# eragonruan/text-detection-ctpn

Hardware: AMD Instinct MI355X
Metric: images/sec at 600x900 (VGG16-CTPN inference) (higher is better)
Workload: dtype bf16

## Files before the change

text-detection-ctpn_amd/csrc/conv3x3_impl.h:

```cpp
#pragma once
#include <cstdlib>
#include <mutex>
#include <type_traits>
#include <utility>

#include "common.h"

namespace ctpn {

constexpr int C3_MAX_DEV = CTPN_MAX_DEV;
static inline int c3_device(int& dev) { return current_device(dev); }
static inline int c3_cu_count(int dev, int& ncu) { return device_cu_count(dev, ncu); }
static inline int c3_raise_lds(const void* kern, bool (&done)[C3_MAX_DEV], int dev) { return raise_dynamic_lds(kern, 160 * 1024, done, dev); }

typedef ctpn_f32x16 c3_f32x16;
typedef __attribute__((ext_vector_type(4))) float c3_f32x4;
typedef uint32_t c3_u32x4 __attribute__((ext_vector_type(4)));

template <typename T>
__device__ __forceinline__ void c3_mfma(c3_f32x16& acc, const uint4& w, const uint4& x) {
  if constexpr (std::is_same<T, float>::value) {
    acc = __builtin_amdgcn_mfma_f32_32x32x2f32(__builtin_bit_cast(float, w.x), __builtin_bit_cast(float, x.x), acc, 0, 0, 0);
    acc = __builtin_amdgcn_mfma_f32_32x32x2f32(__builtin_bit_cast(float, w.y), __builtin_bit_cast(float, x.y), acc, 0, 0, 0);
    acc = __builtin_amdgcn_mfma_f32_32x32x2f32(__builtin_bit_cast(float, w.z), __builtin_bit_cast(float, x.z), acc, 0, 0, 0);
// ... 865 lines not shown
          const uint32_t offA = (uint32_t)((wm * (Wo + 2) + xa) * opitch) * 2u;
          store_pair(pb + (size_t)offA, rok && (cur.x0 >> 1) + xa < Wo, pb + (size_t)offA + (size_t)(8 * opitch) * 2u, rok && (cur.x0 >> 1) + xb < Wo, true, mine);
        } else {
          const int Xl = lq >> 1;
          const uint32_t loff = (uint32_t)((wm * (Wo + 2) + Xl) * opitch) * (uint32_t)sizeof(OutT);
          store_tile(pb + (size_t)loff, !odd && (cur.y0 >> 1) + wm < Ho && (cur.x0 >> 1) + Xl < Wo && ch0 < g.Co, mine);
        }
      } else if constexpr (TW == 32) {
        c3_f32x16 v0, v1;
#pragma unroll
        for (int r = 0; r < 16; ++r) { v0[r] = __builtin_fmaxf(acc[0][0][r], acc[0][1][r]); v1[r] = __builtin_fmaxf(acc[NTL - 1][0][r], acc[NTL - 1][1][r]); }
        hpool(v0, v1, wm, lq >> 1, true);
      } else {
        const int vpart = ((lane & 32) | ((lq & 16) ? ((lq - 2) & 15) : 16 + ((lq + 2) & 15))) << 2;
#pragma unroll
        for (int j = 0; j < MT; ++j) {
          c3_f32x16 v0, v1;
#pragma unroll
          for (int r = 0; r < 16; ++r) {
            const float a0 = acc[0][j][r], a1 = acc[NTL - 1][j][r];
            float b0 = __builtin_bit_cast(float, __builtin_amdgcn_ds_bpermute(vpart, __builtin_bit_cast(int, a0)));
            float b1 = __builtin_bit_cast(float, __builtin_amdgcn_ds_bpermute(vpart, __builtin_bit_cast(int, a1)));
            asm volatile("" : "+v"(b0), "+v"(b1));
            v0[r] = __builtin_fmaxf(a0, b0); v1[r] = __builtin_fmaxf(a1, b1);
          }
          hpool(v0, v1, wm * MT + j, (lq & 15) >> 1, (lq & 16) == 0);
        }
      }
    }
    if (!has_next) break;
    lid = nlid;
    cur = nxt;
    cur_tile = nxt_tile; cur_half = nxt_half;
    if constexpr (HT) active = cur_half < 0 || wm < 2;
  }
  c3_wait_vm<0>();
}

struct Conv3WR {
  const void* in; const void* wt; const float* bias; void* out; void* pool_out;
  int N, H, W, Co;
  int tiles_x, tiles_y, tiles_n;
  unsigned ptiles;
  unsigned groups, per_group;
  unsigned magic_img, magic_row;
  char* dump;
  unsigned* claim;
  const void* q; const void* wfq;
  int Hq, Wq;
};

constexpr int WR_PITCH = 144, WR_PW = 34, WR_ROWS = 10 * WR_PW, WR_PIECES = 48, WR_WIN = WR_PIECES * 1024, WR_NBUF = 3, WR_PD = 8;
static_assert(WR_ROWS * WR_PITCH <= WR_WIN, "window must fit its pieces");

template <int... I, typename F>
__device__ __forceinline__ void c3_static_for_impl(std::integer_sequence<int, I...>, F&& f) { (f(std::integral_constant<int, I>{}), ...); }
template <int N, typename F>
__device__ __forceinline__ void c3_static_for(F&& f) { c3_static_for_impl(std::make_integer_sequence<int, N>{}, f); }

template <int OFF, bool XA = false>
__device__ __forceinline__ void c3_ds_read_b128_off(c3_u32x4& dst, uint32_t lds_addr) {
  if constexpr (XA) asm volatile("ds_read_b128 %0, %1 offset:%2" : "+a"(dst) : "v"(lds_addr), "n"(OFF));
  else asm volatile("ds_read_b128 %0, %1 offset:%2" : "+v"(dst) : "v"(lds_addr), "n"(OFF));
}
#define C3_DEFINE_SLOTS(SFX, MN, XC) \
template <int OFF, int WAIT, int INIT> \
__device__ __forceinline__ void c3_slot1##SFX(c3_f32x16& a0, const c3_u32x4& w0, c3_u32x4& x, uint32_t xaddr, const c3_f32x16& bias) { \
  if constexpr (INIT == 0) \
    asm volatile("s_waitcnt lgkmcnt(%6)\n\t" MN "%0, %2, %1, %3\n\tds_read_b128 %1, %4 offset:%5" \
                 : "+v"(a0), XC(x) : "a"(w0), "v"(bias), "v"(xaddr), "n"(OFF), "n"(WAIT)); \
  else \
    asm volatile("s_waitcnt lgkmcnt(%5)\n\t" MN "%0, %2, %1, %0\n\tds_read_b128 %1, %3 offset:%4" \
                 : "+v"(a0), XC(x) : "a"(w0), "v"(xaddr), "n"(OFF), "n"(WAIT)); \
} \
template <int OFF, int WAIT, int INIT> \
__device__ __forceinline__ void c3_slot2##SFX(c3_f32x16& a0, c3_f32x16& a1, const c3_u32x4& w0, const c3_u32x4& w1, c3_u32x4& x, uint32_t xaddr, \
                                         const c3_f32x16& bias) { \
  if constexpr (INIT == 0) \
    asm volatile("s_waitcnt lgkmcnt(%8)\n\t" MN "%0, %3, %2, %5\n\t" MN "%1, %4, %2, %1\n\tds_read_b128 %2, %6 offset:%7" \
                 : "+v"(a0), "+v"(a1), XC(x) : "a"(w0), "a"(w1), "v"(bias), "v"(xaddr), "n"(OFF), "n"(WAIT)); \
  else if constexpr (INIT == 1) \
    asm volatile("s_waitcnt lgkmcnt(%8)\n\t" MN "%0, %3, %2, %0\n\t" MN "%1, %4, %2, %5\n\tds_read_b128 %2, %6 offset:%7" \
                 : "+v"(a0), "+v"(a1), XC(x) : "a"(w0), "a"(w1), "v"(bias), "v"(xaddr), "n"(OFF), "n"(WAIT)); \
  else \
    asm volatile("s_waitcnt lgkmcnt(%7)\n\t" MN "%0, %3, %2, %0\n\t" MN "%1, %4, %2, %1\n\tds_read_b128 %2, %5 offset:%6" \
                 : "+v"(a0), "+v"(a1), XC(x) : "a"(w0), "a"(w1), "v"(xaddr), "n"(OFF), "n"(WAIT)); \
} \
template <int OFF, int WAIT> \
__device__ __forceinline__ void c3_slot3##SFX(c3_f32x16& a0, c3_f32x16& a1, c3_f32x16& a2, const c3_u32x4& w0, const c3_u32x4& w1, const c3_u32x4& w2, \
                                         c3_u32x4& x, uint32_t xaddr) { \
  asm volatile("s_waitcnt lgkmcnt(%9)\n\t" MN "%0, %4, %3, %0\n\t" MN "%1, %5, %3, %1\n\t" MN "%2, %6, %3, %2\n\tds_read_b128 %3, %7 offset:%8" \
               : "+v"(a0), "+v"(a1), "+v"(a2), XC(x) : "a"(w0), "a"(w1), "a"(w2), "v"(xaddr), "n"(OFF), "n"(WAIT)); \
}
C3_DEFINE_SLOTS(_bf16, "v_mfma_f32_32x32x16_bf16 ", "+v")
C3_DEFINE_SLOTS(_f16, "v_mfma_f32_32x32x16_f16 ", "+v")
C3_DEFINE_SLOTS(_bf16a, "v_mfma_f32_32x32x16_bf16 ", "+a")
C3_DEFINE_SLOTS(_f16a, "v_mfma_f32_32x32x16_f16 ", "+a")
#undef C3_DEFINE_SLOTS
template <bool F16, bool XA, int OFF, int WAIT, int INIT>
__device__ __forceinline__ void c3_slot1(c3_f32x16& a0, const c3_u32x4& w0, c3_u32x4& x, uint32_t xaddr, const c3_f32x16& bias) {
  if constexpr (F16 && XA) c3_slot1_f16a<OFF, WAIT, INIT>(a0, w0, x, xaddr, bias);
  else if constexpr (F16) c3_slot1_f16<OFF, WAIT, INIT>(a0, w0, x, xaddr, bias);
  else if constexpr (XA) c3_slot1_bf16a<OFF, WAIT, INIT>(a0, w0, x, xaddr, bias);
  else c3_slot1_bf16<OFF, WAIT, INIT>(a0, w0, x, xaddr, bias);
}
template <bool F16, bool XA, int OFF, int WAIT, int INIT>
// ... 44 lines not shown
  return w > 15 ? 15 : w;
}

__host__ __device__ constexpr int fq_slot_of(int kind, int id) {
  for (int n = 0; n < 72; ++n)
    if ((kind == 0 ? fq_setup(n) : kind == 1 ? fq_read(n) : kind == 2 ? fq_mma(n) : fq_epi(n)) == id) return n;
  return -1;
}
__host__ __device__ constexpr bool fq_schedule_ok() {
  for (int n = 0; n < 72; ++n) {
    if (fq_lds_ops(n) > 1) return false;
    if ((fq_setup(n) >= 0 || fq_lds_ops(n) || fq_mma(n) >= 0) && (n <= WR_PD || n > 69)) return false;
  }
  if (!(FQ_INCOMING > WR_PD + 8 && FQ_DMA > FQ_INCOMING && FQ_DMA < WR_PD + 1 + 12)) return false;
  for (int gi = 0; gi < 3; ++gi) {
    if (fq_slot_of(0, gi) < 0 || fq_slot_of(0, gi) >= fq_slot_of(1, gi * 3)) return false;
    for (int ky = 0; ky < 3; ++ky) {
      const int r = fq_slot_of(1, gi * 3 + ky);
      if (r < 0) return false;
      for (int i = 0; i < 2; ++i) {
        const int m = fq_slot_of(2, (gi * 2 + i) * 3 + ky);
        if (m < r + 9) return false;
        if (ky > 0 && m <= fq_slot_of(2, (gi * 2 + i) * 3 + ky - 1)) return false;
      }
      if (gi + 2 < 3 && (fq_slot_of(1, (gi + 2) * 3 + ky) < fq_slot_of(2, (gi * 2 + 1) * 3 + ky) || fq_slot_of(0, gi + 2) <= fq_slot_of(1, gi * 3 + 2))) return false;
    }
    for (int i = 0; i < 2; ++i)
      for (int h = 0; h < 4; ++h) {
        const int e = fq_slot_of(3, (gi * 2 + i) * 4 + h);
        if (e < fq_slot_of(2, (gi * 2 + i) * 3 + 2) + 2) return false;
        if (gi + 1 < 3 && fq_slot_of(2, ((gi + 1) * 2 + i) * 3) < e) return false;
      }
  }
  return true;
}
static_assert(fq_schedule_ok(), "producer schedule violates one of its invariants");

typedef uint32_t c3_u32x2 __attribute__((ext_vector_type(2)));
template <int O0, int O1>
__device__ __forceinline__ void c3_fq_read2(c3_u32x4& dst, uint32_t addr) {
  asm volatile("ds_read2_b64 %0, %1 offset0:%2 offset1:%3" : "+a"(dst) : "v"(addr), "n"(O0), "n"(O1));
}
template <bool F16, bool FIRST>
__device__ __forceinline__ void c3_fq_mfma(c3_f32x16& acc, const c3_u32x4& w, const c3_u32x4& x) {
  if constexpr (FIRST) {
    if constexpr (F16) asm volatile("v_mfma_f32_32x32x16_f16 %0, %1, %2, 0" : "+v"(acc) : "a"(w), "a"(x));
    else asm volatile("v_mfma_f32_32x32x16_bf16 %0, %1, %2, 0" : "+v"(acc) : "a"(w), "a"(x));
  } else {
    if constexpr (F16) asm volatile("v_mfma_f32_32x32x16_f16 %0, %1, %2, %0" : "+v"(acc) : "a"(w), "a"(x));
    else asm volatile("v_mfma_f32_32x32x16_bf16 %0, %1, %2, %0" : "+v"(acc) : "a"(w), "a"(x));
  }
}
template <int OFF>
__device__ __forceinline__ void c3_fq_write(uint32_t addr, const c3_u32x2& d) {
  asm volatile("ds_write_b64 %0, %1 offset:%2" : : "v"(addr), "v"(d), "n"(OFF) : "memory");
}
template <typename HF, bool POOL, bool FULL, int ABL = 0, bool FUSE = false>
__global__ __launch_bounds__(256, 1) void conv3x3_wr_kernel(Conv3WR g) {
  constexpr bool F16 = std::is_same<HF, h_f16>::value;
  static_assert(POOL || FULL, "nothing to store");
  static_assert(!FUSE || (POOL && !FULL && ABL == 0), "the fused form is conv1_2's production launch");
  constexpr int PD = WR_PD;
  extern __shared__ __attribute__((aligned(16))) char smem[];
  const uint32_t lds0 = (uint32_t)(uintptr_t)(__attribute__((address_space(3))) char*)smem;
  const int tid = threadIdx.x, lane = tid & 63;
  const int wave = __builtin_amdgcn_readfirstlane(tid >> 6);
  const int ph = wave & 1, chh = wave >> 1;
  const int l31 = lane & 31, fhalf = lane >> 5;
  const int H = g.H, W = g.W, Co = g.Co, Wp = W + 2, Hp = H + 2;
  const int tiles_n = g.tiles_n, tiles_x = g.tiles_x;
  const unsigned per_img = (unsigned)(g.tiles_x * g.tiles_y);
  const unsigned magic_img = g.magic_img, magic_row = g.magic_row;
  const unsigned grp = blockIdx.x % g.groups, kq = blockIdx.x / g.groups;
  const int tn = (int)(kq % (unsigned)tiles_n);
  const int n0 = tn * 64 + chh * 32;
  const unsigned worker = kq / (unsigned)tiles_n, nworkers = gridDim.x / (g.groups * (unsigned)tiles_n);
  const unsigned range_lo = grp * g.per_group;
  const unsigned ptiles = range_lo + g.per_group < g.ptiles ? range_lo + g.per_group : g.ptiles;
  const char* const in_base = (const char*)g.in;

  c3_u32x4 wf[9][4];
  {
    const char* wp = (const char*)g.wt + (size_t)(n0 + l31) * (9 * 64 * 2) + fhalf * 16;
#pragma unroll
    for (int t = 0; t < 9; ++t)
#pragma unroll
      for (int q = 0; q < 4; ++q) wf[t][q] = *(const c3_u32x4*)(wp + t * 128 + q * 32);
  }
  c3_f32x16 bias16;
#pragma unroll
  for (int g4 = 0; g4 < 4; ++g4) {
    const c3_f32x4 b4 = *(const c3_f32x4*)(g.bias + n0 + 8 * g4 + 4 * fhalf);
#pragma unroll
    for (int e = 0; e < 4; ++e) bias16[4 * g4 + e] = b4[e];
  }

  uint32_t voff[FUSE ? 1 : 12];
  if constexpr (!FUSE) {
#pragma unroll
    for (int i = 0; i < 12; ++i) {
      const int o = (wave + 4 * i) * 1024 + lane * 16;
      int row = o / WR_PITCH;
      int slot = (o - row * WR_PITCH) >> 4;
      if (row >= WR_ROWS || slot == 8) { row = 0; slot = 0; }
      const int i2 = row / WR_PW, j2 = row - i2 * WR_PW;
      voff[i] = (uint32_t)((i2 * Wp + j2) * 128 + slot * 16);
    }
  }
  uint32_t fq_rd[3] = {0u, 0u, 0u}, fq_rc[3] = {0u, 0u, 0u}, fq_wr = 0u;
  c3_u32x4 wq[6];
  if constexpr (FUSE) {
#pragma unroll
    for (int gi = 0; gi < 3; ++gi) {
      const int p = 85 * wave + fq_goff(gi) + l31;
// ... 52 lines not shown
      for (int k = 0; k < 3; ++k) xq[a][k] = c3_u32x4{0u, 0u, 0u, 0u};
      pacc[a] = c3_f32x16{0.f, 0.f, 0.f, 0.f, 0.f, 0.f, 0.f, 0.f, 0.f, 0.f, 0.f, 0.f, 0.f, 0.f, 0.f, 0.f};
    }
  }
  auto fq_setup_piece = [&](auto gic, int y2, int x2, uint32_t plane_off) {
    constexpr int gi = decltype(gic)::value;
    const uint32_t r = fq_rc[gi] & 0xffu, c = fq_rc[gi] >> 8;
    const bool in = (r + (uint32_t)(y2 - 1)) < (uint32_t)H && (c + (uint32_t)(x2 - 1)) < (uint32_t)W;
    fq_a[gi & 1] = in ? fq_rd[gi] + plane_off : lds0 + (uint32_t)FQ_ZERO_OFF;
  };
  auto fq_read_piece = [&](auto gic, auto kyc) {
    constexpr int gi = decltype(gic)::value, ky = decltype(kyc)::value;
    c3_fq_read2<ky * FQ_PW, ky * FQ_PW + 1>(xq[gi & 1][ky], fq_a[gi & 1]);
  };
  auto fq_mma_piece = [&](auto gic, auto ic, auto kyc) {
    constexpr int gi = decltype(gic)::value, i = decltype(ic)::value, ky = decltype(kyc)::value;
    c3_fq_mfma<F16, ky == 0>(pacc[i], wq[i * 3 + ky], xq[gi & 1][ky]);
  };
  auto fq_epi_piece = [&](auto gic, auto ic, auto hc, uint32_t wbuf) {
    constexpr int gi = decltype(gic)::value, i = decltype(ic)::value, h = decltype(hc)::value;
    typedef short s16x2 __attribute__((ext_vector_type(2)));
    auto rp = [](uint32_t u) -> uint32_t { return __builtin_bit_cast(uint32_t, __builtin_elementwise_max(__builtin_bit_cast(s16x2, u), s16x2{0, 0})); };
    c3_u32x2 d;
    d[0] = rp(c3_cvt_pk<HF>(pacc[i][4 * h], pacc[i][4 * h + 1]));
    d[1] = rp(c3_cvt_pk<HF>(pacc[i][4 * h + 2], pacc[i][4 * h + 3]));
    c3_fq_write<fq_goff(gi) * WR_PITCH + 64 * i + 16 * h>(wbuf, d);
  };
  auto fq_produce_sync = [&](unsigned pt, int plane, uint32_t wbuf) {
    int img, y2, x2;
    tile_coords(pt, img, y2, x2);
    c3_static_for<3>([&](auto gic) {
      fq_setup_piece(gic, y2, x2, (uint32_t)(plane * FQ_PLANE));
      c3_static_for<3>([&](auto kyc) { fq_read_piece(gic, kyc); });
      c3_wait_lgkm<0>();
      c3_static_for<2>([&](auto ic) {
        c3_static_for<3>([&](auto kyc) { fq_mma_piece(gic, ic, kyc); });
      });
      asm volatile("s_nop 15\n\ts_nop 15" ::: "memory");
      __builtin_amdgcn_sched_barrier(0);
      c3_static_for<2>([&](auto ic) {
        c3_static_for<4>([&](auto hc) { fq_epi_piece(gic, ic, hc, wbuf); });
      });
      __builtin_amdgcn_sched_barrier(0);
    });
  };

  unsigned* claim_ctr;
  {
    const unsigned long long a = (unsigned long long)(uintptr_t)(g.claim + 2 * (grp * (unsigned)tiles_n + (unsigned)tn));
    const unsigned lo = sgpr((unsigned)a), hi = sgpr((unsigned)(a >> 32));
    claim_ctr = (unsigned*)(uintptr_t)(((unsigned long long)hi << 32) | lo);
  }
  const unsigned claim_base = sgpr(range_lo + 5u * nworkers);
  const uint32_t claim_lds = lds0 + WR_NBUF * WR_WIN;
  auto claim_issue = [&](uint32_t& ret) {
    if (wave == 0 && lane == 0) {
      const uint32_t zero = 0u, one = 1u;
      asm volatile("global_atomic_add %0, %1, %2, %3 sc0" : "+a"(ret) : "v"(zero), "a"(one), "s"(claim_ctr) : "memory");
    }
  };
  auto claim_publish = [&](uint32_t& ret, unsigned word) {
    if (wave == 0 && lane == 0) {
      const uint32_t a = claim_lds + 4 * word;
      uint32_t tmp;
      asm volatile("v_accvgpr_read_b32 %0, %1\n\tv_add_u32 %0, %0, %3\n\tds_write_b32 %2, %0" : "=&v"(tmp) : "a"(ret), "v"(a), "s"(claim_base) : "memory");
    }
  };
  auto claim_read = [&](uint32_t& dst, unsigned word) {
    const uint32_t a = claim_lds + 4 * word;
    asm volatile("ds_read_b32 %0, %1" : "+a"(dst) : "v"(a));
  };
  auto claim_value = [&](uint32_t& dst) -> unsigned {
    uint32_t v;
    asm volatile("v_accvgpr_read_b32 %0, %1" : "=v"(v) : "a"(dst));
    return (unsigned)__builtin_amdgcn_readfirstlane((int)v);
  };
  unsigned q0 = range_lo + worker, q1 = q0 + nworkers, q2 = q0 + 2 * nworkers;
  if (q0 >= ptiles) {
    if (tid == 0) {
      const unsigned done = __hip_atomic_fetch_add(claim_ctr + 1, 1u, __ATOMIC_RELAXED, __HIP_MEMORY_SCOPE_AGENT);
      if (done == nworkers - 1) { __hip_atomic_store(claim_ctr, 0u, __ATOMIC_RELAXED, __HIP_MEMORY_SCOPE_AGENT); __hip_atomic_store(claim_ctr + 1, 0u, __ATOMIC_RELAXED, __HIP_MEMORY_SCOPE_AGENT); }
    }
    return;
  }
  if constexpr (!FUSE) {
    const char* b0 = window_base(q0);
    const char* b1 = window_base(q1 < ptiles ? q1 : q0);
    c3_static_for<12>([&](auto ic) { issue_piece(ic, b0, lds0); });
    c3_static_for<12>([&](auto ic) { issue_piece(ic, b1, lds0 + WR_WIN); });
  } else {
    {
      const uint32_t za = lds0 + (uint32_t)FQ_ZERO_OFF + 4u * (uint32_t)tid, zero = 0u;
      asm volatile("ds_write_b32 %0, %1" : : "v"(za), "v"(zero) : "memory");
    }
    const char* const pb0 = q_base(q0);
    const char* const pb1 = q_base(q1 < ptiles ? q1 : q0);
    const char* const pb2 = q_base(q2 < ptiles ? q2 : q0);
    asm volatile("s_nop 4" ::: "memory");
    issue_plane(pb0, 0);
    issue_plane(pb1, 1);
    c3_wait_vm<0>();
    c3_wait_lgkm<0>();
    c3_barrier();
    fq_produce_sync(q0, 0, fq_wr);
    fq_produce_sync(q1 < ptiles ? q1 : q0, 1, fq_wr + (uint32_t)WR_WIN);
    c3_wait_lgkm<0>();
    c3_barrier();
    issue_plane(pb2, 0);
  }
  const uint32_t xbase = lds0 + (uint32_t)((4 * ph * WR_PW + l31) * WR_PITCH + fhalf * 16);
  c3_wait_vm<0>();
  if constexpr (FUSE) c3_wait_lgkm<0>();
  c3_barrier();

  c3_u32x4 xr[PD];
  c3_f32x16 acc[2][4];
#pragma unroll
  for (int i = 0; i < PD; ++i) xr[i] = c3_u32x4{0u, 0u, 0u, 0u};
#pragma unroll
  for (int a = 0; a < 2; ++a)
#pragma unroll
    for (int j = 0; j < 4; ++j) acc[a][j] = bias16;
// ... 39 lines not shown
      const int Ho = H >> 1, Wo = W >> 1;
      const int Ys = (y0 >> 1) + 2 * ph, Xs = x0 >> 1;
      const unsigned pix = sgpr((unsigned)((img * (Ho + 2) + Ys + 1) * (Wo + 2) + Xs + 1));
      const c3_gptr rb = sbase64(g.pool_out, ((unsigned long long)pix << co_shift) + (unsigned)(n0 * 2));
      c3_u32x4 v[2];
#pragma unroll
      for (int q = 0; q < 2; ++q) {
        const auto r0 = __builtin_amdgcn_permlane32_swap(pk[4 * q + 0], pk[4 * q + 2], false, false);
        const auto r1 = __builtin_amdgcn_permlane32_swap(pk[4 * q + 1], pk[4 * q + 3], false, false);
        v[q] = c3_u32x4{r0[0], r1[0], r0[1], r1[1]};
      }
      c3_u32x4 va, vb;
#pragma unroll
      for (int c = 0; c < 4; ++c) {
        const auto r = __builtin_amdgcn_permlane16_swap(v[0][c], v[1][c], false, false);
        va[c] = r[0]; vb[c] = r[1];
      }
      const bool rowok = valid && Ys + (odd ? 1 : 0) < Ho;
      const int xa = (l31 & 15) >> 1;
      const c3_gptr da = rowok && Xs + xa < Wo ? rb + (size_t)pool_pair_off : dump_lane;
      const c3_gptr db = rowok && Xs + 8 + xa < Wo ? rb + (size_t)pool_pair_off + (size_t)(8 * Co * 2) : dump_lane;
      *(__attribute__((address_space(1))) c3_u32x4*)(da) = va;
      *(__attribute__((address_space(1))) c3_u32x4*)(db) = vb;
    }
  };
  const uint32_t full_pair_off = (uint32_t)((l31 & 15) * Co * 2 + (2 * ((lane >> 4) & 1) + fhalf) * 16);
  auto full_piece = [&](auto esc, auto jc, auto qc, int img, int y0, int x0, bool valid) {
    constexpr int es = decltype(esc)::value, j = decltype(jc)::value, q2 = decltype(qc)::value;
#pragma unroll
    for (int h = 0; h < 4; ++h) pk[4 * q2 + h] = relu_pk(c3_cvt_pk<HF>(acc[es][j][8 * q2 + 2 * h], acc[es][j][8 * q2 + 2 * h + 1]));
    if constexpr (q2 == 1) {
      const int y = y0 + 4 * ph + j;
      const unsigned pix = sgpr((unsigned)((img * Hp + y + 1) * Wp + x0 + 1));
      const c3_gptr rb = sbase64(g.out, ((unsigned long long)pix << co_shift) + (unsigned)(n0 * 2));
      c3_u32x4 v[2];
#pragma unroll
      for (int q = 0; q < 2; ++q) {
        const auto r0 = __builtin_amdgcn_permlane32_swap(pk[4 * q + 0], pk[4 * q + 2], false, false);
        const auto r1 = __builtin_amdgcn_permlane32_swap(pk[4 * q + 1], pk[4 * q + 3], false, false);
        v[q] = c3_u32x4{r0[0], r1[0], r0[1], r1[1]};
      }
      c3_u32x4 va, vb;
#pragma unroll
      for (int c = 0; c < 4; ++c) {
        const auto r = __builtin_amdgcn_permlane16_swap(v[0][c], v[1][c], false, false);
        va[c] = r[0]; vb[c] = r[1];
      }
      const bool rowok = valid && y < H;
      const c3_gptr da = rowok && x0 + (l31 & 15) < W ? rb + (size_t)full_pair_off : dump_lane;
      const c3_gptr db = rowok && x0 + 16 + (l31 & 15) < W ? rb + (size_t)full_pair_off + (size_t)(16 * Co * 2) : dump_lane;
      *(__attribute__((address_space(1))) c3_u32x4*)(da) = va;
      *(__attribute__((address_space(1))) c3_u32x4*)(db) = vb;
    }
  };
  constexpr int NE = (POOL ? 18 : 0) + (FULL ? 8 : 0);
  constexpr int NS = (POOL ? 2 : 0) + (FULL ? 8 : 0);
  constexpr int D_FIRST = PD + 1, E_FIRST = D_FIRST + 12, E_STRIDE = (64 - E_FIRST) / NE;
  static_assert(E_STRIDE >= 1 && E_FIRST + (NE - 1) * E_STRIDE <= 63, "epilogue pieces must fit the tile's slots");
  auto epi_piece = [&](auto esc, auto ec, int img, int y0, int x0, bool valid) {
    constexpr int e = decltype(ec)::value;
    if constexpr (POOL && e < 18) {
      if constexpr (e == 8) pool_store(std::integral_constant<int, 0>{}, img, y0, x0, valid);
      else if constexpr (e == 17) pool_store(std::integral_constant<int, 1>{}, img, y0, x0, valid);
      else pool_elem(esc, std::integral_constant<int, (e < 8 ? e : e - 1)>{});
    } else {
      constexpr int f = e - (POOL ? 18 : 0);
      full_piece(esc, std::integral_constant<int, f / 2>{}, std::integral_constant<int, f % 2>{}, img, y0, x0, valid);
    }
  };

  uint32_t claim_ret = 0u, claim_val = 0u;
  unsigned bcur = 0, bnext = 1, bdma = 2;
  auto tile = [&](auto asc, unsigned k) {
    constexpr int as = decltype(asc)::value;
    k = sgpr(k);
    int c_img, c_y0, c_x0;
    tile_coords(q0, c_img, c_y0, c_x0);
    const char* nbase = nullptr;
    int n_img = 0, n_y0 = 0, n_x0 = 0;
    if constexpr (FUSE) tile_coords(q2 < ptiles ? q2 : q0, n_img, n_y0, n_x0);
    else nbase = window_base(q2 < ptiles ? q2 : q0);
    const uint32_t nbuf_lds = sgpr(lds0 + bdma * WR_WIN);
    const uint32_t fq_wbuf = fq_wr + sgpr(bdma * WR_WIN);
    const uint32_t xcur = xbase + sgpr(bcur * WR_WIN);
    const uint32_t xnext = xbase + sgpr((q1 < ptiles ? bnext : bcur) * WR_WIN);
    unsigned incoming = 0u;
    const char* dma_base = nullptr;
    c3_static_for<72>([&](auto nc) {
      constexpr int n = decltype(nc)::value;
      constexpr int r = wr_slot_r(n), kx = wr_slot_kx(n), q = wr_slot_q(n);
      if constexpr (n == PD) {
        c3_wait_vm<(ABL & 2) ? 0 : NS>();
        c3_barrier();
        claim_read(claim_val, (k + 1) & 1);
        claim_publish(claim_ret, k & 1);
        claim_issue(claim_ret);
      }
      constexpr int nn = (n + PD) % 72;
      constexpr int off = wr_slot_off(nn);
      constexpr int WT = FUSE ? fq_wait(n) : PD - 1;
      const uint32_t xa = (n + PD < 72) ? xcur : xnext;
      constexpr int j_lo = r - 2 < 0 ? 0 : r - 2, j_hi = r > 3 ? 3 : r;
      constexpr int nm = j_hi - j_lo + 1;
      if constexpr (nm == 1) {
        constexpr int ky = r - j_hi;
        c3_slot1<F16, FUSE, off, WT, wr_first_touch(n, ky) ? 0 : -1>(acc[as][j_hi], wf[ky * 3 + kx][q], xr[n % PD], xa, bias16);
      } else if constexpr (nm == 2) {
        constexpr int ky0 = r - j_hi, ky1 = ky0 + 1;
        constexpr int init = wr_first_touch(n, ky0) ? 0 : (wr_first_touch(n, ky1) ? 1 : -1);
        c3_slot2<F16, FUSE, off, WT, init>(acc[as][j_hi], acc[as][j_hi - 1], wf[ky0 * 3 + kx][q], wf[ky1 * 3 + kx][q], xr[n % PD], xa, bias16);
      } else {
        static_assert(!wr_first_touch(n, 0) && !wr_first_touch(n, 1) && !wr_first_touch(n, 2), "three-row slots never start a chain");
        constexpr int ky0 = r - j_hi;
        c3_slot3<F16, FUSE, off, WT>(acc[as][j_hi], acc[as][j_hi - 1], acc[as][j_hi - 2], wf[ky0 * 3 + kx][q], wf[(ky0 + 1) * 3 + kx][q], wf[(ky0 + 2) * 3 + kx][q],
                                     xr[n % PD], xa);
      }
      if constexpr (!FUSE) {
        if constexpr (n >= D_FIRST && n < D_FIRST + 12 && !(ABL & 1)) issue_piece(std::integral_constant<int, n - D_FIRST>{}, nbase, nbuf_lds);
      } else {
        if constexpr (fq_setup(n) >= 0) fq_setup_piece(std::integral_constant<int, fq_setup(n)>{}, n_y0, n_x0, (uint32_t)(as * FQ_PLANE));
        if constexpr (fq_epi(n) >= 0)
          fq_epi_piece(std::integral_constant<int, fq_epi(n) / 8>{}, std::integral_constant<int, (fq_epi(n) / 4) % 2>{}, std::integral_constant<int, fq_epi(n) % 4>{}, fq_wbuf);
        if constexpr (fq_mma(n) >= 0)
          fq_mma_piece(std::integral_constant<int, fq_mma(n) / 6>{}, std::integral_constant<int, (fq_mma(n) / 3) % 2>{}, std::integral_constant<int, fq_mma(n) % 3>{});
        if constexpr (fq_read(n) >= 0) fq_read_piece(std::integral_constant<int, fq_read(n) / 3>{}, std::integral_constant<int, fq_read(n) % 3>{});
        if constexpr (n == FQ_INCOMING) {
          incoming = sgpr(k < 2 ? range_lo + worker + (k + 3) * nworkers : claim_value(claim_val));
          dma_base = q_base(incoming < ptiles ? incoming : q0);
        }
        if constexpr (n == FQ_DMA) issue_plane(dma_base, as ^ 1);
      }
      if constexpr (n >= E_FIRST && (n - E_FIRST) % E_STRIDE == 0 && (n - E_FIRST) / E_STRIDE < NE && !(ABL & 2))
        epi_piece(std::integral_constant<int, as ^ 1>{}, std::integral_constant<int, (n - E_FIRST) / E_STRIDE>{}, p_img, p_y0, p_x0, p_valid);
      __builtin_amdgcn_sched_barrier(0);
    });
    p_img = c_img; p_y0 = c_y0; p_x0 = c_x0; p_valid = true;
    if constexpr (!FUSE) incoming = k < 2 ? range_lo + worker + (k + 3) * nworkers : claim_value(claim_val);
    q0 = q1; q1 = q2; q2 = sgpr(incoming);
    const unsigned b = bcur; bcur = bnext; bnext = bdma; bdma = b;
  };

  unsigned k = 0;
  bool last_set1 = false;
  for (;;) {
    tile(std::integral_constant<int, 0>{}, k);
    last_set1 = false;
    if (q0 >= ptiles) break;
    tile(std::integral_constant<int, 1>{}, k + 1);
    last_set1 = true;
    if (q0 >= ptiles) break;
    k += 2;
  }
  c3_wait_lgkm<0>();
  if (!last_set1) c3_static_for<NE>([&](auto ec) { epi_piece(std::integral_constant<int, 0>{}, ec, p_img, p_y0, p_x0, true); });
  else c3_static_for<NE>([&](auto ec) { epi_piece(std::integral_constant<int, 1>{}, ec, p_img, p_y0, p_x0, true); });
  c3_wait_vm<0>();
  if (tid == 0) {
    const unsigned done = __hip_atomic_fetch_add(claim_ctr + 1, 1u, __ATOMIC_RELAXED, __HIP_MEMORY_SCOPE_AGENT);
    if (done == nworkers - 1) {
      __hip_atomic_store(claim_ctr, 0u, __ATOMIC_RELAXED, __HIP_MEMORY_SCOPE_AGENT);
      __hip_atomic_store(claim_ctr + 1, 0u, __ATOMIC_RELAXED, __HIP_MEMORY_SCOPE_AGENT);
    }
  }
}

int c3_wr_resources(int dev, hipStream_t s, char** dump, unsigned** claim);

template <typename H>
static int c3_launch_wr(const Conv3& c, bool pool, hipStream_t s) {
  Conv3WR g{};
  g.in = c.in; g.wt = c.wt; g.bias = c.bias; g.out = c.out; g.pool_out = c.pool_out;
  g.N = c.N; g.H = c.H; g.W = c.W; g.Co = c.Co;
  int he, we;
  {
    he = (pool && !c.out) ? (c.H & ~1) : c.H;
    we = (pool && !c.out) ? (c.W & ~1) : c.W;
    if (c.w_cover > 0 && c.w_cover < we) we = c.w_cover;
  }
  g.tiles_x = (we + 31) / 32;
  g.tiles_y = (he + 7) / 8;
  g.tiles_n = c.Co / 64;
  const long long ptiles = (long long)c.N * g.tiles_x * g.tiles_y;
  const long long per_img = (long long)g.tiles_x * g.tiles_y;
  if (ptiles <= 0 || ptiles * per_img >= (1LL << 32) || (long long)c.N * (c.H + 2) * (c.W + 2) * 128 >= (1LL << 40))
    return fail(CTPN_ERR_ARG, "conv3x3_wr: problem out of range");
  g.ptiles = (unsigned)ptiles;
  g.magic_img = (unsigned)((1ULL << 32) / (unsigned long long)per_img + 1ULL);
  g.magic_row = (unsigned)((1ULL << 32) / (unsigned long long)g.tiles_x + 1ULL);
  int dev = 0, ncu = 0, rc;
  if ((rc = c3_device(dev)) || (rc = c3_cu_count(dev, ncu))) return rc;
  g.groups = 8u;
  g.per_group = (unsigned)((ptiles + g.groups - 1) / g.groups);
  long long workers = (ncu / g.tiles_n) / (long long)g.groups;
  if (workers < 1) workers = 1;
  if (workers > (long long)g.per_group) workers = g.per_group;
  workers *= g.groups;
  if (workers * g.tiles_n > 1024) return fail(CTPN_ERR_ARG, "conv3x3_wr: more workgroups than dump pages");
  if (g.tiles_n > 4) return fail(CTPN_ERR_ARG, "conv3x3_wr: more channel slices than claim counters per slot");
  if ((rc = c3_wr_resources(dev, s, &g.dump, &g.claim))) return rc;
  const bool fuse = c.q1 != nullptr;
  if (fuse) {
    if (!pool || c.out || c.Co != 64 || !c.q1_frags) return fail(CTPN_ERR_ARG, "conv3x3_wr: the fused conv1_1 form is conv1_2's pooled production launch");
    g.q = c.q1; g.wfq = c.q1_frags; g.Hq = conv1_q_h(c.H); g.Wq = conv1_q_w(c.W);
    if (8 * g.tiles_y + 4 > g.Hq || 32 * g.tiles_x + 4 > g.Wq || (long long)c.N * g.Hq * g.Wq >= (1LL << 31))
      return fail(CTPN_ERR_ARG, "conv3x3_wr: q-image geometry out of range");
  }
  const int lds = fuse ? FQ_LDS : WR_NBUF * WR_WIN + 16;
  const dim3 grid((unsigned)(workers * g.tiles_n)), block(256);
  static bool attr[10][C3_MAX_DEV] = {{false}};
  auto launch = [&](auto kern, bool (&done)[C3_MAX_DEV]) -> int {
    const int r = c3_raise_lds((const void*)kern, done, dev);
    if (r) return r;
    hipLaunchKernelGGL(kern, grid, block, lds, s, g);
    return CTPN_OK;
  };
#ifdef CTPN_ABLATION
  static const int var = [] { const char* e = std::getenv("CTPN_C3_WR_VAR"); return e ? std::atoi(e) : 0; }();
#else
  constexpr int var = 0;
#endif
  if (fuse) rc = launch(conv3x3_wr_kernel<H, true, false, 0, true>, attr[9]);
  else if (pool && c.out) rc = launch(conv3x3_wr_kernel<H, true, true>, attr[0]);
  else if (pool) {
    switch (var) {
#ifdef CTPN_ABLATION
      case 1: rc = launch(conv3x3_wr_kernel<H, true, false, 1>, attr[1]); break;
      case 2: rc = launch(conv3x3_wr_kernel<H, true, false, 2>, attr[2]); break;
      case 3: rc = launch(conv3x3_wr_kernel<H, true, false, 3>, attr[3]); break;
#endif
      default: rc = launch(conv3x3_wr_kernel<H, true, false>, attr[4]);
    }
  } else {
    switch (var) {
#ifdef CTPN_ABLATION
      case 1: rc = launch(conv3x3_wr_kernel<H, false, true, 1>, attr[5]); break;
      case 2: rc = launch(conv3x3_wr_kernel<H, false, true, 2>, attr[6]); break;
      case 3: rc = launch(conv3x3_wr_kernel<H, false, true, 3>, attr[7]); break;
#endif
      default: rc = launch(conv3x3_wr_kernel<H, false, true>, attr[8]);
    }
  }
  if (rc) return rc;
  hipError_t e = hipGetLastError();
  if (e != hipSuccess) return fail(CTPN_ERR_HIP, std::string("conv3x3_wr launch: ") + hipGetErrorString(e));
  return CTPN_OK;
}

static inline void c3_extent(const Conv3& g, bool pool, int& he, int& we) {
  he = (pool && !g.out) ? (g.H & ~1) : g.H;
  we = (pool && !g.out) ? (g.W & ~1) : g.W;
  if (g.w_cover > 0 && g.w_cover < we) we = g.w_cover;
}
static inline long long c3_tiles2d(const Conv3& g, bool pool, int tw) {
  int he, we;
  c3_extent(g, pool, he, we);
  const int th = C3_BM / tw;
  return (long long)((we + tw - 1) / tw) * ((he + th - 1) / th);
}

template <typename T, typename OutT, int BN, int WGM, int WGN, bool FLAT, bool POOL, int ABUF, int NBUF, int TW = 32, bool SPLIT = false>
static int c3_launch(Conv3 g, hipStream_t s) {
  constexpr int C3_TW = TW, C3_TH = C3_BM / TW, C3_PW2D = C3_TW + 2;
  constexpr int NTHR = WGM * WGN * 64;
  constexpr int EP = BN * (int)sizeof(OutT) + 16;
  const int Wp = g.W + 2;
  const int rows = FLAT ? (C3_BM + 2 * Wp + 2) : (C3_TH + 2) * C3_PW2D;
  g.a_rows = (rows + 7) & ~7;
  constexpr int NWL = WGM * WGN;
  constexpr int AG_MAX = FLAT ? (61 + NWL - 1) / NWL : (43 + NWL - 1) / NWL;
  if ((g.a_rows >> 3) > AG_MAX * NWL) return fail(CTPN_ERR_ARG, "conv3x3: input window does not fit the flat-mode staging plan");
  g.tiles_n = (g.Co + BN - 1) / BN;
  long long ptiles;
  if (FLAT) {
    g.m_total = (long long)g.N * (g.H + 2) * Wp;
    ptiles = (g.m_total + C3_BM - 1) / C3_BM;
  } else {
    int he, we;
    c3_extent(g, POOL, he, we);
    g.tiles_x = (we + C3_TW - 1) / C3_TW;
    g.tiles_y = (he + C3_TH - 1) / C3_TH;
    ptiles = (long long)g.N * g.tiles_x * g.tiles_y;
  }
  const long long nblk = ptiles * g.tiles_n;
  if (nblk <= 0 || nblk > 0x7fffffffLL) return fail(CTPN_ERR_ARG, "conv3x3: grid out of range");
  const int main_lds = ABUF * g.a_rows * 128 + NBUF * BN * 128;
  const int epi_lds = C3_BM * EP;
  const int lds = main_lds > epi_lds ? main_lds : epi_lds;
  if (lds > 160 * 1024) return fail(CTPN_ERR_ARG, "conv3x3: LDS budget exceeded");
  auto k = conv3x3_kernel<T, OutT, BN, WGM, WGN, FLAT, POOL, ABUF, NBUF, TW, SPLIT>;
  static bool attr[C3_MAX_DEV] = {false};
  int dev = 0, rc;
  if ((rc = c3_device(dev)) || (rc = c3_raise_lds((const void*)k, attr, dev))) return rc;
// ... 331 lines not shown
```

Baseline: 3706.

## Exchange half-rows between waves through LDS for contiguous full-output stores

```diff
diff --git a/text-detection-ctpn_amd/csrc/conv3x3_impl.h b/text-detection-ctpn_amd/csrc/conv3x3_impl.h
--- a/text-detection-ctpn_amd/csrc/conv3x3_impl.h
+++ b/text-detection-ctpn_amd/csrc/conv3x3_impl.h
@@ -941,6 +941,8 @@
 
 constexpr int WR_PITCH = 144, WR_PW = 34, WR_ROWS = 10 * WR_PW, WR_PIECES = 48, WR_WIN = WR_PIECES * 1024, WR_NBUF = 3, WR_PD = 8;
 static_assert(WR_ROWS * WR_PITCH <= WR_WIN, "window must fit its pieces");
+constexpr int WR_TAIL = WR_ROWS * WR_PITCH, WR_XCH_OFF = WR_NBUF * WR_WIN, WR_XCH_LDS = WR_XCH_OFF + 4 * 4096;
+static_assert(WR_TAIL + 8 <= WR_WIN && WR_XCH_LDS <= 160 * 1024, "queue words / exchange buffer");
 
 template <int... I, typename F>
 __device__ __forceinline__ void c3_static_for_impl(std::integer_sequence<int, I...>, F&& f) { (f(std::integral_constant<int, I>{}), ...); }
@@ -1091,6 +1093,10 @@
   }
 }
 template <int OFF>
+__device__ __forceinline__ void c3_xch_write(uint32_t addr, const c3_u32x4& d) {
+  asm volatile("ds_write_b128 %0, %1 offset:%2" : : "v"(addr), "v"(d), "n"(OFF) : "memory");
+}
+template <int OFF>
 __device__ __forceinline__ void c3_fq_write(uint32_t addr, const c3_u32x2& d) {
   asm volatile("ds_write_b64 %0, %1 offset:%2" : : "v"(addr), "v"(d), "n"(OFF) : "memory");
 }
@@ -1099,6 +1105,7 @@
   constexpr bool F16 = std::is_same<HF, h_f16>::value;
   static_assert(POOL || FULL, "nothing to store");
   static_assert(!FUSE || (POOL && !FULL && ABL == 0), "the fused form is conv1_2's production launch");
+  constexpr bool XCH = FULL && !POOL;
   constexpr int PD = WR_PD;
   extern __shared__ __attribute__((aligned(16))) char smem[];
   const uint32_t lds0 = (uint32_t)(uintptr_t)(__attribute__((address_space(3))) char*)smem;
@@ -1257,22 +1264,20 @@
     claim_ctr = (unsigned*)(uintptr_t)(((unsigned long long)hi << 32) | lo);
   }
   const unsigned claim_base = sgpr(range_lo + 5u * nworkers);
-  const uint32_t claim_lds = lds0 + WR_NBUF * WR_WIN;
+  const uint32_t claim_lds = lds0 + (XCH ? WR_TAIL : WR_NBUF * WR_WIN);
   auto claim_issue = [&](uint32_t& ret) {
     if (wave == 0 && lane == 0) {
       const uint32_t zero = 0u, one = 1u;
       asm volatile("global_atomic_add %0, %1, %2, %3 sc0" : "+a"(ret) : "v"(zero), "a"(one), "s"(claim_ctr) : "memory");
     }
   };
-  auto claim_publish = [&](uint32_t& ret, unsigned word) {
+  auto claim_publish = [&](uint32_t& ret, uint32_t a) {
     if (wave == 0 && lane == 0) {
-      const uint32_t a = claim_lds + 4 * word;
       uint32_t tmp;
       asm volatile("v_accvgpr_read_b32 %0, %1\n\tv_add_u32 %0, %0, %3\n\tds_write_b32 %2, %0" : "=&v"(tmp) : "a"(ret), "v"(a), "s"(claim_base) : "memory");
     }
   };
-  auto claim_read = [&](uint32_t& dst, unsigned word) {
-    const uint32_t a = claim_lds + 4 * word;
+  auto claim_read = [&](uint32_t& dst, uint32_t a) {
     asm volatile("ds_read_b32 %0, %1" : "+a"(dst) : "v"(a));
   };
   auto claim_value = [&](uint32_t& dst) -> unsigned {
@@ -1418,6 +1423,95 @@
       *(__attribute__((address_space(1))) c3_u32x4*)(da) = va;
       *(__attribute__((address_space(1))) c3_u32x4*)(db) = vb;
     }
+  };
+  uint32_t xch_w = 0u, xch_r = 0u, xch_off[2] = {0u, 0u};
+  c3_u32x4 xrecv[2];
+  const bool xb3 = (lane & 8) != 0;
+  if constexpr (XCH) {
+    xch_w = lds0 + (uint32_t)(WR_XCH_OFF + wave * 4096 + lane * 16);
+    xch_r = lds0 + (uint32_t)(WR_XCH_OFF + (wave ^ 2) * 4096 + (lane ^ 8) * 16);
+    const int piece = 2 * ((lane >> 4) & 1) + fhalf;
+#pragma unroll
+    for (int sI = 0; sI < 2; ++sI)
+      xch_off[sI] = (uint32_t)((16 * chh + 8 * sI + (lane & 7)) * Co * 2 + (4 * (xb3 == (sI != 0) ? chh : 1 - chh) + piece) * 16);
+    xrecv[0] = c3_u32x4{0u, 0u, 0u, 0u}; xrecv[1] = c3_u32x4{0u, 0u, 0u, 0u};
+  }
+  auto full_row = [&](auto esc, auto jc, c3_u32x4& va, c3_u32x4& vb) {
+    constexpr int es = decltype(esc)::value, j = decltype(jc)::value;
+    uint32_t p[8];
+#pragma unroll
+    for (int h = 0; h < 8; ++h) p[h] = relu_pk(c3_cvt_pk<HF>(acc[es][j][2 * h], acc[es][j][2 * h + 1]));
+    c3_u32x4 v[2];
+#pragma unroll
+    for (int q = 0; q < 2; ++q) {
+      const auto r0 = __builtin_amdgcn_permlane32_swap(p[4 * q + 0], p[4 * q + 2], false, false);
+      const auto r1 = __builtin_amdgcn_permlane32_swap(p[4 * q + 1], p[4 * q + 3], false, false);
+      v[q] = c3_u32x4{r0[0], r1[0], r0[1], r1[1]};
+    }
+#pragma unroll
+    for (int c = 0; c < 4; ++c) {
+      const auto r = __builtin_amdgcn_permlane16_swap(v[0][c], v[1][c], false, false);
+      va[c] = r[0]; vb[c] = r[1];
+    }
+  };
+  auto full_give = [&](auto esc, auto jc) {
+    constexpr int j = decltype(jc)::value;
+    c3_u32x4 va, vb;
+    full_row(esc, jc, va, vb);
+    c3_u32x4 gv;
+#pragma unroll
+    for (int c = 0; c < 4; ++c) gv[c] = chh ? va[c] : vb[c];
+    c3_xch_write<j * 1024>(xch_w, gv);
+  };
+  auto full_fetch = [&](auto jc) {
+    constexpr int j = decltype(jc)::value;
+    c3_ds_read_b128_off<j * 1024, true>(xrecv[j & 1], xch_r);
+  };
+  auto full_store = [&](auto esc, auto jc, int img, int y0, int x0, bool valid) {
+    constexpr int j = decltype(jc)::value;
+    c3_u32x4 va, vb;
+    full_row(esc, jc, va, vb);
+    asm volatile("" : "+a"(xrecv[j & 1]));
+    const c3_u32x4 rv = xrecv[j & 1];
+    c3_u32x4 d0, d1;
+#pragma unroll
+    for (int c = 0; c < 4; ++c) {
+      const uint32_t kp = chh ? vb[c] : va[c];
+      d0[c] = xb3 ? rv[c] : kp;
+      d1[c] = xb3 ? kp : rv[c];
+    }
+    const int y = y0 + 4 * ph + j;
+    const unsigned pix = sgpr((unsigned)((img * Hp + y + 1) * Wp + x0 + 1));
+    const c3_gptr rb = sbase64(g.out, ((unsigned long long)pix << co_shift) + (unsigned)(tn * 128));
+    const bool rowok = valid && y < H;
+    const int xp = x0 + 16 * chh + (lane & 7);
+    const c3_gptr da = rowok && xp < W ? rb + (size_t)xch_off[0] : dump_lane;
+    const c3_gptr db = rowok && xp + 8 < W ? rb + (size_t)xch_off[1] : dump_lane;
+    *(__attribute__((address_space(1))) c3_u32x4*)(da) = d0;
+    *(__attribute__((address_space(1))) c3_u32x4*)(db) = d1;
+  };
+  constexpr int XCH_G0 = PD + 2, XCH_MB = 32, XCH_S0 = XCH_MB + 8;
+  auto xch_slot = [&](auto esc, auto nc, int img, int y0, int x0, bool valid) {
+    constexpr int n = decltype(nc)::value;
+    if constexpr (n >= XCH_G0 && n < XCH_G0 + 16 && (n - XCH_G0) % 4 == 0) full_give(esc, std::integral_constant<int, (n - XCH_G0) / 4>{});
+    if constexpr (n == XCH_MB) full_fetch(std::integral_constant<int, 0>{});
+    if constexpr (n == XCH_MB + 4) full_fetch(std::integral_constant<int, 1>{});
+    if constexpr (n >= XCH_S0 && n < XCH_S0 + 16 && (n - XCH_S0) % 4 == 0) {
+      constexpr int j = (n - XCH_S0) / 4;
+      full_store(esc, std::integral_constant<int, j>{}, img, y0, x0, valid);
+      if constexpr (j + 2 < 4) full_fetch(std::integral_constant<int, j + 2>{});
+    }
+  };
+  auto xch_drain = [&](auto esc, int img, int y0, int x0) {
+    c3_barrier();
+    c3_static_for<4>([&](auto jc) { full_give(esc, jc); });
+    c3_wait_lgkm<0>();
+    c3_barrier();
+    c3_static_for<4>([&](auto jc) {
+      full_fetch(jc);
+      c3_wait_lgkm<0>();
+      full_store(esc, jc, img, y0, x0, true);
+    });
   };
   constexpr int NE = (POOL ? 18 : 0) + (FULL ? 8 : 0);
   constexpr int NS = (POOL ? 2 : 0) + (FULL ? 8 : 0);
@@ -1458,9 +1552,13 @@
       if constexpr (n == PD) {
         c3_wait_vm<(ABL & 2) ? 0 : NS>();
         c3_barrier();
-        claim_read(claim_val, (k + 1) & 1);
-        claim_publish(claim_ret, k & 1);
+        claim_read(claim_val, claim_lds + 4 * ((k + 1) & 1) + (XCH ? sgpr(bcur * WR_WIN) : 0u));
+        claim_publish(claim_ret, claim_lds + 4 * (k & 1) + (XCH ? sgpr(bnext * WR_WIN) : 0u));
         claim_issue(claim_ret);
+      }
+      if constexpr (XCH && !(ABL & 2) && n == XCH_MB) {
+        c3_wait_lgkm<0>();
+        c3_barrier();
       }
       constexpr int nn = (n + PD) % 72;
       constexpr int off = wr_slot_off(nn);
@@ -1496,7 +1594,9 @@
         }
         if constexpr (n == FQ_DMA) issue_plane(dma_base, as ^ 1);
       }
-      if constexpr (n >= E_FIRST && (n - E_FIRST) % E_STRIDE == 0 && (n - E_FIRST) / E_STRIDE < NE && !(ABL & 2))
+      if constexpr (XCH) {
+        if constexpr (!(ABL & 2)) xch_slot(std::integral_constant<int, as ^ 1>{}, nc, p_img, p_y0, p_x0, p_valid);
+      } else if constexpr (n >= E_FIRST && (n - E_FIRST) % E_STRIDE == 0 && (n - E_FIRST) / E_STRIDE < NE && !(ABL & 2))
         epi_piece(std::integral_constant<int, as ^ 1>{}, std::integral_constant<int, (n - E_FIRST) / E_STRIDE>{}, p_img, p_y0, p_x0, p_valid);
       __builtin_amdgcn_sched_barrier(0);
     });
@@ -1518,8 +1618,13 @@
     k += 2;
   }
   c3_wait_lgkm<0>();
-  if (!last_set1) c3_static_for<NE>([&](auto ec) { epi_piece(std::integral_constant<int, 0>{}, ec, p_img, p_y0, p_x0, true); });
-  else c3_static_for<NE>([&](auto ec) { epi_piece(std::integral_constant<int, 1>{}, ec, p_img, p_y0, p_x0, true); });
+  if constexpr (XCH) {
+    if (!last_set1) xch_drain(std::integral_constant<int, 0>{}, p_img, p_y0, p_x0);
+    else xch_drain(std::integral_constant<int, 1>{}, p_img, p_y0, p_x0);
+  } else {
+    if (!last_set1) c3_static_for<NE>([&](auto ec) { epi_piece(std::integral_constant<int, 0>{}, ec, p_img, p_y0, p_x0, true); });
+    else c3_static_for<NE>([&](auto ec) { epi_piece(std::integral_constant<int, 1>{}, ec, p_img, p_y0, p_x0, true); });
+  }
   c3_wait_vm<0>();
   if (tid == 0) {
     const unsigned done = __hip_atomic_fetch_add(claim_ctr + 1, 1u, __ATOMIC_RELAXED, __HIP_MEMORY_SCOPE_AGENT);
@@ -1574,10 +1679,10 @@
   const int lds = fuse ? FQ_LDS : WR_NBUF * WR_WIN + 16;
   const dim3 grid((unsigned)(workers * g.tiles_n)), block(256);
   static bool attr[10][C3_MAX_DEV] = {{false}};
-  auto launch = [&](auto kern, bool (&done)[C3_MAX_DEV]) -> int {
+  auto launch = [&](auto kern, bool (&done)[C3_MAX_DEV], int lds_bytes) -> int {
     const int r = c3_raise_lds((const void*)kern, done, dev);
     if (r) return r;
-    hipLaunchKernelGGL(kern, grid, block, lds, s, g);
+    hipLaunchKernelGGL(kern, grid, block, lds_bytes, s, g);
     return CTPN_OK;
   };
 #ifdef CTPN_ABLATION
@@ -1585,25 +1690,25 @@
 #else
   constexpr int var = 0;
 #endif
-  if (fuse) rc = launch(conv3x3_wr_kernel<H, true, false, 0, true>, attr[9]);
-  else if (pool && c.out) rc = launch(conv3x3_wr_kernel<H, true, true>, attr[0]);
+  if (fuse) rc = launch(conv3x3_wr_kernel<H, true, false, 0, true>, attr[9], lds);
+  else if (pool && c.out) rc = launch(conv3x3_wr_kernel<H, true, true>, attr[0], lds);
   else if (pool) {
     switch (var) {
 #ifdef CTPN_ABLATION
-      case 1: rc = launch(conv3x3_wr_kernel<H, true, false, 1>, attr[1]); break;
-      case 2: rc = launch(conv3x3_wr_kernel<H, true, false, 2>, attr[2]); break;
-      case 3: rc = launch(conv3x3_wr_kernel<H, true, false, 3>, attr[3]); break;
+      case 1: rc = launch(conv3x3_wr_kernel<H, true, false, 1>, attr[1], lds); break;
+      case 2: rc = launch(conv3x3_wr_kernel<H, true, false, 2>, attr[2], lds); break;
+      case 3: rc = launch(conv3x3_wr_kernel<H, true, false, 3>, attr[3], lds); break;
 #endif
-      default: rc = launch(conv3x3_wr_kernel<H, true, false>, attr[4]);
+      default: rc = launch(conv3x3_wr_kernel<H, true, false>, attr[4], lds);
     }
   } else {
     switch (var) {
 #ifdef CTPN_ABLATION
-      case 1: rc = launch(conv3x3_wr_kernel<H, false, true, 1>, attr[5]); break;
-      case 2: rc = launch(conv3x3_wr_kernel<H, false, true, 2>, attr[6]); break;
-      case 3: rc = launch(conv3x3_wr_kernel<H, false, true, 3>, attr[7]); break;
+      case 1: rc = launch(conv3x3_wr_kernel<H, false, true, 1>, attr[5], WR_XCH_LDS); break;
+      case 2: rc = launch(conv3x3_wr_kernel<H, false, true, 2>, attr[6], WR_XCH_LDS); break;
+      case 3: rc = launch(conv3x3_wr_kernel<H, false, true, 3>, attr[7], WR_XCH_LDS); break;
 #endif
-      default: rc = launch(conv3x3_wr_kernel<H, false, true>, attr[8]);
+      default: rc = launch(conv3x3_wr_kernel<H, false, true>, attr[8], WR_XCH_LDS);
     }
   }
   if (rc) return rc;
```

New measurement: 3710, median of 3. Within noise of the previous version (+0.1%).
